# hdm0922/PathTracerDemo

Hardware: AMD Instinct MI355X
Metric: Msamples/sec at 1920x1080, 1 spp ReSTIR DI; per-pixel L2 vs WebGPU ref (higher is better)
Workload: dtype f32; 1 GPU; c3_interior_32 reuse 1920x1080, 1 spp/frame (configs[2]); frame=1920x1080, band_rows_per_gpu=1080, parallelism=row-bands x1

## Files before the change

### pathtracerdemo_amd/csrc/ptx_api.cpp

```cpp
#include <hip/hip_runtime.h>

#include <algorithm>
#include <cmath>
#include <cstdarg>
#include <cstdlib>
#include <cstdio>
#include <cstring>
#include <new>
#include <string>
#include <unordered_map>
#include <vector>

#include "ptx_internal.h"

namespace ptx {


[[maybe_unused]] static const char *const kShippedKnobs[] = {"COMM_TIMEOUT_S", "DEBUG_FILL", "HALO_PROXY_US"};
#if defined(PTX_WG_TIMES)
static const char *const kBuildKind = "wgt";
#elif defined(PTX_AB_BUILD)
static const char *const kBuildKind = "ab";
#else
static const char *const kBuildKind = "product";
// ... 758 lines not shown
                if (e != hipSuccess) break;
            }
            TimedLaunch *t = event_begin(h, PTX_STAT_WAVE_LOGIC, st);
            e = wave_gi_round(sc, w, gp, r, A, st);
            event_end(t, st);
        }
        return e;
    }
    if (pass == PTX_PASS_TEMPORAL || pass == PTX_PASS_SPATIAL || pass == kPassTemporalJobs ||
        pass == kPassTemporalCombine || is_motion_pass(pass)) {
        const bool temporal = pass != PTX_PASS_SPATIAL;
        ReuseArgs A = is_motion_pass(pass) ? motion_args(h)
                                           : reuse_args(h, temporal ? PTX_PASS_TEMPORAL : PTX_PASS_SPATIAL);
        WaveBufs wj = w;
        if (A.fold_last && wj.res[2]) wj.nres = 3;
        else A.fold_last = 0u;
        if (fused && pass == PTX_PASS_SPATIAL) {
            A.fuse_final = 1u;
            A.accum = (float4 *)h->d_accum.p;
            A.replay_cnt = (uint32_t *)h->d_replay.p;
            A.replay = A.replay_cnt + w.cnt_stride;
            A.replay_total = (unsigned long long *)h->d_counters.p + CNT_REPLAY;
        }
        const int nr = reuse_rounds(temporal, A);
        const int r_first = pass == kPassTemporalCombine ? nr + 1 : 0;
        const int r_last = pass == kPassTemporalJobs ? nr : nr + 1;
        for (int r = r_first; e == hipSuccess && r <= r_last; ++r) {
            if (r > 0 && r <= nr) {
                TimedLaunch *t = event_begin(h, PTX_STAT_WAVE_TRACE, st);
                e = wave_trace(sc, wj, r - 1, 1, h->stack_depth, st);
                event_end(t, st);
            }
            if (e != hipSuccess) break;
            if (r == nr && A.fold_last) continue;
            const bool combine = r == nr + 1 && pass == PTX_PASS_SPATIAL;
            if (combine && combine_after && (e = hipStreamWaitEvent(st, combine_after, 0)) != hipSuccess) break;
            TimedLaunch *t = event_begin(h, PTX_STAT_WAVE_LOGIC, st);
            e = wave_reuse_round(sc, wj, temporal, r, A, st);
            event_end(t, st);
            if (combine && combine_done && e == hipSuccess) e = hipEventRecord(combine_done, st);
        }
        return e;
    }
    const uint4 *fres = h->cfg.pipeline == PTX_PIPELINE_RESTIR_REUSE ? (const uint4 *)hist_band(h) : res;
    static const bool final_one = ab_knob("FINAL_ONE", 1) != 0;
    if (pass == PTX_PASS_FINAL && final_one && h->cfg.pipeline == PTX_PIPELINE_RESTIR_REUSE && tables_fit_lds(sc)) {
        TimedLaunch *t = event_begin(h, PTX_STAT_WAVE_LOGIC, st);
        if (fused)
            e = wave_final_replay(sc, w, gb, fres, acc, (const uint32_t *)h->d_replay.p + w.cnt_stride,
                                  (uint32_t *)h->d_replay.p, h->stack_depth, st);
        else
            e = wave_final_one(sc, w, gb, fres, acc, h->stack_depth, st);
        event_end(t, st);
        h->launches[PTX_STAT_FINAL_FUSED] += 1;
        h->cur().init_state_valid = false;
        return e;
    }
    h->cur().init_state_valid = pass == PTX_PASS_INIT && h->cfg.pipeline == PTX_PIPELINE_RESTIR_REUSE;
    const int rounds = pass == PTX_PASS_INIT ? kWaveRoundsInit : pass == PTX_PASS_FINAL ? kWaveRoundsFinal
                                                                                        : kWaveRoundsMcpt;
    for (int r = 0; e == hipSuccess && r <= rounds; ++r) {
        if (r > 0) {
            TimedLaunch *t = event_begin(h, PTX_STAT_WAVE_TRACE, st);
            e = wave_trace(sc, w, r - 1, 1, h->stack_depth, st);
            event_end(t, st);
        }
        if (e != hipSuccess) break;
// ... 59 lines not shown
    static const int env_bk = ab_knob("PIPE_BACK_STREAMS", 2);
    int k = env_bk > 0 && frames_in_flight(h) ? env_bk : 1;
    if (h->cfg.flags & PTX_FLAG_SINGLE_STREAM) k = 1;
    k = std::max(1, std::min<int>({k, ptx_handle::kMaxSplit, (int)interior.nseg, (int)edge.nseg}));
    ReuseArgs A = reuse_args(h, PTX_PASS_SPATIAL);
    const bool fold = A.fold_last && interior.res[2];
    if (!fold) A.fold_last = 0u;
    const int nr = reuse_rounds(0, A);
    if ((e = fork_sequences(h, k)) != hipSuccess) return e;
    const bool surf_stale = interior.surf && !h->cur().surf_valid;
    uint32_t E = 0u;
    for (int q = 0; q < k && e == hipSuccess; ++q) {
        hipStream_t st = q ? h->cur().sub[q] : h->cur().stream;
        WaveBufs wi = interior, we = edge;
        seg_share(wi, interior.nseg, q, k);
        seg_share(we, edge.nseg, q, k);
        wi.seg_phys = interior.seg_phys + E;
        we.seg_phys = interior.seg_phys + E + wi.seg_base + wi.seg_count - we.seg_base;
        E += we.seg_count;
        if (fold) wi.nres = we.nres = 3;
        WaveBufs wt = wi;
        wt.seg_count = wi.seg_count + we.seg_count;
        if (surf_stale) {
            if ((e = wave_surface(sc, wi, gbuf_band(h), st)) != hipSuccess) return e;
            if ((e = wave_surface(sc, we, gbuf_band(h), st)) != hipSuccess) return e;
        }
        for (int r = 0; e == hipSuccess && r <= nr + 1; ++r) {
            if (r > 0 && r <= nr) {
                TimedLaunch *t = event_begin(h, PTX_STAT_WAVE_TRACE, st);
                e = wave_trace(sc, wt, r - 1, 1, h->stack_depth, st);
                event_end(t, st);
                if (e != hipSuccess) break;
            }
            if (r == nr && A.fold_last) continue;
            TimedLaunch *t = event_begin(h, PTX_STAT_WAVE_LOGIC, st);
            e = wave_reuse_round(sc, wi, 0, r, A, st);
            if (e == hipSuccess && r == 0 && halo) e = hipStreamWaitEvent(st, halo, 0);
            if (e == hipSuccess) e = wave_reuse_round(sc, we, 0, r, A, st);
            event_end(t, st);
        }
        for (const WaveBufs *ws : {&wi, &we})
            if (e == hipSuccess) e = launch_wave_seq(h, sc, *ws, PTX_PASS_FINAL, st);
    }
    if (surf_stale && e == hipSuccess) h->cur().surf_valid = true;
    return e == hipSuccess ? join_sequences(h, k) : e;
}

hipError_t launch_wave_parts(ptx_handle *h, const Scene &sc, const WaveBufs &w, const int *passes, int npasses,
                             bool summaries, const WaveBufs *then, hipEvent_t then_wait, bool keep_gbuf) {
    h->hand_n = 0;
    static const bool overlap_start = ab_knob("OVERLAP_START", 1) != 0;
    if (then && overlap_start && npasses == 2 && passes[0] == PTX_PASS_SPATIAL && passes[1] == PTX_PASS_FINAL &&
        h->cfg.pipeline == PTX_PIPELINE_RESTIR_REUSE && !summaries)
        return spatial_overlap_seq(h, sc, w, *then, then_wait);
    static const int env_k = ab_knob("WAVE_STREAMS", 0);
    static const int env_pk = ab_knob("PIPE_STREAMS", 0);
    const bool band_h = h->comm || h->halo_top || h->halo_bot || (h->cfg.flags & PTX_FLAG_HALO_SKIP);
    const int pipe_k = env_pk > 0 ? env_pk : band_h || h->cfg.pipeline == PTX_PIPELINE_RESTIR_GI ? 1 : 2;
    int k = frames_in_flight(h) ? pipe_k : env_k > 0 ? env_k : 3;
    static const int env_bk = ab_knob("PIPE_BACK_STREAMS", 2);
    if (env_bk > 0 && frames_in_flight(h))
        for (int i = 0; i < npasses; ++i)
            if (passes[i] == PTX_PASS_SPATIAL) k = env_bk;
    if (h->cfg.flags & PTX_FLAG_SINGLE_STREAM) k = 1;
    k = std::max(1, std::min<int>(k, ptx_handle::kMaxSplit));
    if ((uint32_t)k > std::max(w.nseg, then ? then->nseg : 0u)) k = (int)std::max(w.nseg, then ? then->nseg : 0u);
    hipError_t e = hipSuccess;
// ... 2187 lines not shown
```

### pathtracerdemo_amd/csrc/ptx_reuse.hip

```cpp
#include "ptx_wave_common.h"

namespace ptx {

constexpr uint32_t SALT_TEMPORAL = 0x54454D50u, SALT_SPATIAL = 0x53504154u;

enum : uint32_t { JS_HDR, JS_F, JS_CUR, JS_NRM, JS_PREV, JS_RRF, JS_COUNT };
constexpr uint32_t kJobFresh = 1u << 24;
constexpr uint32_t kResReuseLayout = 0x100u;
#ifndef PTX_JOB_FRESH
#define PTX_JOB_FRESH 1
#endif

struct Job {
    uint32_t i, length, phase, seed1, idx, matref;
    uint32_t k, lab;
    bool shift, rok;
    int32_t ref;
    int32_t dom;
    f3 f;
    float prod;
    Surface cur;
    f3 prev;
    float beta, rr_p;
    f3 rr_f;
// ... 321 lines not shown
}
__device__ __forceinline__ float4 job_at(const ReuseArgs &A, const WaveBufs &w, uint32_t pix, uint32_t slot) {
    const uint32_t jid = job_id(A, pix, slot);
    return job_result(A, w, A.jres[jid], jid);
}
__device__ __forceinline__ SelF stored_f(const uint4 *r) {
    const uint4 r6 = r[6], r7 = r[7];
    return SelF{r7.w == 1u, mk(asf(r6.z), asf(r6.w), asf(r7.z))};
}
__device__ __forceinline__ uint32_t write_reused(uint4 *out, const uint4 *src, float p_sel, float q_sel, SelF fs,
                                                 float w_sum, uint32_t C) {
    uint4 a0 = src[0], a5 = src[5];
    const uint4 a1 = src[1], a2 = src[2], a3 = src[3], a4 = src[4];
    if (fs.known && !(a5.x & kResReuseLayout)) {
        const uint32_t k = a5.x & 0xffu;
        if (k >= 2u && k + 1u < a5.w) a0 = src[6];
        a5.x |= kResReuseLayout;
    }
    out[0] = a0; out[1] = a1; out[2] = a2; out[3] = a3; out[4] = a4; out[5] = a5;
    out[6] = make_uint4(asu(p_sel), asu(q_sel), fs.known ? asu(fs.f.x) : 0u, fs.known ? asu(fs.f.y) : 0u);
    out[7] = make_uint4(asu(p_sel > 0.0f ? w_sum / p_sel : 0.0f), C, fs.known ? asu(fs.f.z) : 0u, fs.known ? 1u : 0u);
    return a5.w;
}

constexpr uint32_t kNbrEscape = 0xFFFFFFFFu;
__device__ __forceinline__ uint4 nbr_pack(bool valid, uint4 r5, uint4 r6, uint4 r7) {
    uint32_t w = 0u;
    const uint32_t k = r5.x & 0xffu;
    if (valid)
        w = (r5.w > 0xfu || k > 0xfu || r7.y > 0x7ffffeu) ? kNbrEscape : (1u << 31) | (r5.w << 27) | (k << 23) | r7.y;
    return make_uint4(r6.x, r6.y, r7.x, w);
}

__device__ __forceinline__ bool temporal_from_init(const Scene &sc, const WaveBufs &w, const ReuseArgs &A, Job &s,
                                                   uint32_t pix, uint32_t jid) {
    const uint4 *rv = res_at(A.cur, s.ref);
    const bool hyb = job_hyb(s);
    while (s.i + 1u < s.length) {
        f3 V = normalize(s.prev - s.cur.pos);
        uint32_t seed = s.i == 1u ? rv[0].x : s.seed1, lobe;
        const f3 dir = sample_bsdf(seed, s.cur, V, lobe);
        float pdf;
        const f3 fv = bsdf_pdf(s.cur, V, dir, pdf);
        if (!hyb || s.i + 2u <= s.k) s.prod *= pdf;
        if (!rr_step(s, s.cur, dir, fv, pdf)) {
            A.jres[jid] = make_float4(0.0f, 0.0f, 0.0f, 0.0f);
            return false;
        }
        const float4 c = w.state[(s.i == 1u ? kStateCs2 : kStateCs3) * w.npix + pix];
        const Surface next = get_surface(sc, gdecode(make_uint4(asu(c.x), asu(c.y), asu(c.z), asu(c.w))));
        V = normalize(s.prev - s.cur.pos);
        const f3 L = normalize(next.pos - s.cur.pos);
        s.f = s.f * (bsdf(s.cur, L, V) * fabsf(dot(s.cur.nrm, L)));
        if (hyb && s.i + 1u == s.k) s.prod = s.prod * rc_geo(s.cur.pos, next);
        s.prev = s.cur.pos;
        s.cur = next;
        s.i += 1u;
    }
    const float T = w.state[kStateTsel * w.npix + pix].x;
    if (T < 0.0f) return true;
    const LightSample XL = load_xl(rv);
    const f3 V = normalize(s.prev - s.cur.pos);
    const f3 L = direction_to_light(s.cur, XL);
    s.f = s.f * (bsdf(s.cur, L, V) * fabsf(dot(s.cur.nrm, L)));
    float gl = 1.0f;
    if (XL.type == LIGHT_RECT) {
        const f3 r = XL.pos - s.cur.pos;
        const f3 Ld = normalize(r);
        gl = fabsf(dot(get_light(sc, (uint32_t)XL.id).dir, Ld)) / dot(r, r);
    }
    s.prod = hyb ? s.prod / s.beta : s.prod / (gl * s.beta);
    const f3 Le = l_emit<true>(XL, s.cur);
    s.f = s.f * (Le * T);
    const float qv = s.prod;
    const bool valid = qv > 0.0f && qv <= 3.402823466e38f;
    A.jres[jid] = valid ? make_float4(s.f.x, s.f.y, s.f.z, qv) : make_float4(0.0f, 0.0f, 0.0f, 0.0f);
    return false;
}

template <bool LDS_SHADE>
__global__ __launch_bounds__(WB) __attribute__((amdgpu_waves_per_eu(2, 8)))
void wtemporal_start(Scene gsc, WaveBufs w, ReuseArgs A) {
    PTX_WAVE_TIMER(gsc, KID_TEMP_START | (w.seg_base ? 0x80u : 0u));
    __shared__ uint32_t lds[3];
    extern __shared__ __attribute__((aligned(16))) uint32_t shade_lds[];
    const JobLists JL = job_lists(w, lds);
    const Scene sc = shading_scene<LDS_SHADE>(gsc, shade_lds, true);
    const Seg g = seg_begin(w, 0u, lds);
    const uint32_t np = padded_pixels(sc);
    for (uint32_t k = 0; k < w.seg_px; k += WB) {
        const uint32_t q = seg_pixel(w, g.j, k);
        uint32_t x, y, pix = 0u;
        bool active = false;
        Job s;
        if (q < np && tile_xy(sc, q, x, y)) {
            pix = (y - sc.row_begin) * sc.width + x;
            active = job_begin(sc, A, s, x, y, (int32_t)pix, (int32_t)pix);
            if (active && A.use_init) active = temporal_from_init(sc, w, A, s, pix, pix);
        }
        const bool live = job_emit(sc, g, A, active, s, pix, active ? A.cur[8u * (size_t)pix].x : 0u);
        job_finish(g, JL, A, live, s, pix);
    }
    job_seg_end(w, g, JL);
}

__global__ __launch_bounds__(WB) void wtemporal_combine(Scene sc, WaveBufs w, ReuseArgs A) {
    PTX_WAVE_TIMER(sc, KID_TEMP_COMBINE | (w.seg_base ? 0x80u : 0u));
    const uint32_t j = w.seg_base + blockIdx.x, np = padded_pixels(sc);
    for (uint32_t k = 0; k < w.seg_px; k += WB) {
        const uint32_t q = seg_pixel(w, j, k);
        uint32_t x, y;
        if (q >= np || !tile_xy(sc, q, x, y)) continue;
        const uint32_t pix = (y - sc.row_begin) * sc.width + x;
        if (!gdecode(A.gbuf[pix]).valid) {
            A.nbr_out[pix] = make_uint4(0u, 0u, 0u, 0u);
            continue;
        }
        uint4 *rv = A.cur + 8u * (size_t)pix;
        const uint4 *hv = A.hist + 8u * (size_t)pix;
        uint32_t seed = reuse_seed(sc, x, y, SALT_TEMPORAL);
        const uint4 r5 = rv[5], r7 = rv[7];
        const float4 er = (r7.y != 0u && r5.w >= 2u) ? job_result(A, w, A.jres[pix], pix) : make_float4(0.0f, 0.0f, 0.0f, 0.0f);
        const float2 ec = make_float2(er.w > 0.0f ? luminance(mk(er.x, er.y, er.z)) : 0.0f, er.w);
        const bool canon_ok = ec.y > 0.0f && ec.x > 0.0f;
        const uint4 h5 = hv[5], h6 = hv[6], h7 = hv[7];
        const uint32_t Cp = A.hist_valid ? min(h7.y, A.cap) : 0u;
        const float cp = (float)Cp, tot = 1.0f + cp;
        const float pp = asf(h6.x), qp = asf(h6.y);
        const bool hist_ok = Cp != 0u && h5.w >= 2u && pp > 0.0f;
        const float wc = canon_ok ? (1.0f / tot) * ec.x * asf(r7.x) : 0.0f;
        const float wp = hist_ok ? (cp / tot) * pp * asf(h7.x) : 0.0f;
        float w_sum = 0.0f, p_sel = ec.x, q_sel = ec.y;
        bool from_hist = false;
        if (wrs_update(w_sum, wc, seed)) { from_hist = false; p_sel = ec.x; q_sel = ec.y; }
        if (wrs_update(w_sum, wp, seed)) { from_hist = true; p_sel = pp; q_sel = qp; }
        write_reused(rv, from_hist ? hv : rv, p_sel, q_sel, from_hist ? stored_f(hv) : job_f(er), w_sum, 1u + Cp);
// ... 49 lines not shown
template <bool LDS_SHADE>
__global__ __launch_bounds__(WB) __attribute__((amdgpu_waves_per_eu(MOTION_START_WAVES, 8)))
void wtmotion_start(Scene gsc, WaveBufs w, ReuseArgs A) {
    PTX_WAVE_TIMER(gsc, KID_TEMP_START | (w.seg_base ? 0x80u : 0u));
    __shared__ uint32_t lds[3];
    extern __shared__ __attribute__((aligned(16))) uint32_t shade_lds[];
    const JobLists JL = job_lists(w, lds);
    const Scene sc = shading_scene<LDS_SHADE>(gsc, shade_lds, true);
    const Seg g = seg_begin(w, 0u, lds);
    const uint32_t np = padded_pixels(sc);
    for (uint32_t k = 0; k < w.seg_px; k += WB) {
        const uint32_t q = seg_pixel(w, g.j, k);
        uint32_t x = 0u, y = 0u, pix = 0u;
        bool valid = false;
        Surface X1{};
        uint32_t mref = 0u;
        if (q < np && tile_xy(sc, q, x, y)) {
            pix = (y - sc.row_begin) * sc.width + x;
            valid = surf_load(sc, A.surf, pix, X1, mref);
        }
        const uint4 *rv = A.cur + 8u * (size_t)pix;
        const uint4 r5c = valid ? rv[5] : make_uint4(0u, 0u, 0u, 0u);
        const uint32_t cC = valid ? rv[7].y : 0u, clen = r5c.w, ck = r5c.x & 0xffu;
        const bool canon = valid && cC != 0u && clen >= 2u;
        const MotionHist mh = valid ? motion_hist(sc, A, X1, y, true) : MotionHist{false, 0, 0u, 0u, 0u};
#pragma unroll 1
        for (uint32_t slot = 0; slot < kMotionJobs; ++slot) {
            const uint32_t jid = job_id(A, pix, slot);
            Job s;
            bool act = false;
            uint32_t s0 = 0u;
            if (slot == 0u) {
                act = canon && job_begin(sc, A, s, x, y, (int32_t)pix, (int32_t)pix);
                if (act && A.use_init) act = temporal_from_init(sc, w, A, s, pix, jid);
                if (act) s0 = rv[0].x;
            } else if (slot == 1u) {
                if (mh.ok) {
                    const uint4 *hv = A.hist + 8 * (ptrdiff_t)mh.pp;
                    const uint4 h0 = hv[0], h5 = hv[5], h6 = hv[6];
                    act = h5.w >= 2u && asf(h6.x) > 0.0f;
                    if (act) {
                        job_init(s, x0_of(sc, x, y), X1, mref, kHistRef + mh.pp, h5.w, h0.y, (int32_t)pix, h5.x & 0xffu,
                                 true);
                        s0 = h0.x;
                    }
                }
            } else if (mh.ok && canon) {
                Surface Xp;
                uint32_t pref;
                act = surf_load(sc, A.psurf, mh.pp, Xp, pref);
                if (act) {
                    job_init(s, x0_prev(A, sc, mh.px, mh.py), Xp, pref, (int32_t)pix, clen, rv[0].y, kDomPrev, ck, true);
                    s0 = rv[0].x;
                }
            }
            const bool live = job_emit(sc, g, A, act, s, jid, s0);
            job_finish(g, JL, A, live, s, jid);
        }
    }
    job_seg_end(w, g, JL);
}

__global__ __launch_bounds__(WB) void wtmotion_combine(Scene sc, WaveBufs w, ReuseArgs A) {
    PTX_WAVE_TIMER(sc, KID_TEMP_COMBINE | (w.seg_base ? 0x80u : 0u));
    const uint32_t j = w.seg_base + blockIdx.x, np = padded_pixels(sc);
    for (uint32_t k = 0; k < w.seg_px; k += WB) {
        const uint32_t q = seg_pixel(w, j, k);
// ... 502 lines not shown
                if (A.fuse_final) replay = shade_reused(sc, A, t, acc, pix, hit, hit ? Csum : 0u, length, fs, ucw);
            }
        }
        if (A.fuse_final) replay_append(A, w, w.seg_phys + j, replay, pix);
    }
}

__global__ __launch_bounds__(WB) void wspatial_combine(Scene sc, WaveBufs w, ReuseArgs A) {
    PTX_WAVE_TIMER(sc, KID_SPAT_COMBINE | (w.seg_base ? 0x80u : 0u));
    const uint32_t j = w.seg_base + blockIdx.x, np = padded_pixels(sc);
    for (uint32_t k = 0; k < w.seg_px; k += WB) {
        const uint32_t q = seg_pixel(w, j, k);
        uint32_t x, y, pix = 0u;
        bool replay = false;
        if (q < np && tile_xy(sc, q, x, y)) {
            pix = (y - sc.row_begin) * sc.width + x;
            if (!gdecode(A.gbuf[pix]).valid) {
                uint4 *out = A.hist + 8u * (size_t)pix;
                for (int t = 0; t < 8; ++t) out[t] = make_uint4(0u, 0u, 0u, 0u);
                if (A.fuse_final)
                    (void)shade_reused(sc, A, mix_weight(sc), A.accum[pix], pix, false, 0u, 0u,
                                       SelF{false, mk(0.0f, 0.0f, 0.0f)}, 0.0f);
            } else if (A.neighbors == 3u) {
                replay = combine_pixel<3>(sc, A, w, x, y, pix);
            } else {
                replay = combine_pixel<0>(sc, A, w, x, y, pix);
            }
        }
        if (A.fuse_final) replay_append(A, w, w.seg_phys + j, replay, pix);
    }
}

int reuse_rounds(int pass_temporal, const ReuseArgs &A) {
    return pass_temporal && A.use_init && !A.motion ? 1 : kWaveRoundsReuse;
}

hipError_t wave_reuse_round(const Scene &sc, const WaveBufs &w, int pass_temporal, int round, const ReuseArgs &A,
                            hipStream_t s) {
    const dim3 grid(w.seg_count), blk(WB);
    if (round == 0) {
        if (pass_temporal) {
            const bool staged = shade_from_lds(sc, SL_TEMPORAL_START);
            auto k = A.motion ? (staged ? wtmotion_start<true> : wtmotion_start<false>)
                              : (staged ? wtemporal_start<true> : wtemporal_start<false>);
            hipLaunchKernelGGL(k, grid, blk, shade_lds_bytes(staged, sc), s, sc, w, A);
        } else {
            hipLaunchKernelGGL(wspatial_start, grid, blk, 0, s, sc, w, A);
        }
    } else if (round <= reuse_rounds(pass_temporal, A)) {
        const bool staged = shade_from_lds(sc, SL_JOB_STEP);
        auto k = staged ? wjob_step<true> : wjob_step<false>;
        hipLaunchKernelGGL(k, grid, blk, shade_lds_bytes(staged, sc), s, sc, w, (uint32_t)round, A);
    } else {
        if (pass_temporal && A.motion) hipLaunchKernelGGL(wtmotion_combine, grid, blk, 0, s, sc, w, A);
        else if (pass_temporal) hipLaunchKernelGGL(wtemporal_combine, grid, blk, 0, s, sc, w, A);
        else if (A.neighbors == 3u && !ab_knob("COMBINE_SCALAR", 0))
            hipLaunchKernelGGL(wspatial_combine_shfl, dim3(w.seg_count), blk, 0, s, sc, w, A);
        else hipLaunchKernelGGL(wspatial_combine, grid, blk, 0, s, sc, w, A);
    }
    return hipGetLastError();
}

}
```

### pathtracerdemo_amd/csrc/ptx_wave.hip

```cpp
#include "ptx_stream.h"

#include <algorithm>
#include <cstdlib>

namespace ptx {

#ifndef TRACE_OCC_WAVES
#define TRACE_OCC_WAVES 5
#endif
template <bool COUNT, bool PROF, bool OCC, bool LDS_TABLES>
__device__ __forceinline__ void trace_lanes(const Scene &sc, const SubRoot *subs, const Inst *insts, PassEps eps,
                                            uint32_t *stack, CoopLds coop, Ray r, uint32_t kind, float T, float remain,
                                            uint32_t seg, bool active, float4 *res, uint32_t gi) {
    for (;;) {
        const float t_max = !active ? __builtin_nanf("") : kind != Q_CLOSEST ? vis_bound(remain) : 1e10f;
        const Hit h = (LDS_TABLES && !COUNT)
                          ? trace_core_flat<PROF, OCC>(sc, subs, insts, r, eps, stack, WB, t_max, coop, remain)
                          : trace_core_tab<COUNT, PROF, true, OCC, true>(sc, subs, insts, r, eps, stack, WB, t_max, coop,
                                                                         false, remain);
        if (active && end_query(sc, subs, insts, eps, h, r, kind, T, remain, seg, res, gi)) active = false;
        if (wballot(active) == 0ull) break;
    }
}
template <bool COUNT, bool PROF, bool OCC, bool LDS_TABLES>
// ... 165 lines not shown
                sp += 1;
            }
        }
    }
}

template <bool ROOTQ>
__global__ __launch_bounds__(WB) void wgbuffer(Scene sc, WaveBufs w, uint4 *gbuf) {
    PTX_WAVE_TIMER(sc, KID_GBUF);
    extern __shared__ __attribute__((aligned(16))) uint32_t wstack[];
    uint32_t *stack = wstack + tables_lds_bytes(sc) / 4u + threadIdx.x;
    const LdsTables T = stage_tables(sc, wstack);
    const uint32_t L = blockIdx.x * 4u + threadIdx.x / 64u, run = w.cluster * w.seg_count;
    const uint32_t t = set_tile(w, (L / run) * w.cluster * w.nseg + w.cluster * w.seg_base + L % run);
    const uint32_t q = t * 64u + (threadIdx.x & 63u);
    uint32_t x, y;
    if (q >= padded_pixels(sc) || !tile_xy(sc, q, x, y)) return;
    const float *vpinv = reinterpret_cast<const float *>(sc.U + U_VPINV);
    const float u = ((float)x + 0.5f) / (float)sc.U[U_W];
    const float v = ((float)y + 0.5f) / (float)sc.U[U_H];
    const f3 st = xform_point(vpinv, mk(2.0f * u - 1.0f, 2.0f * v - 1.0f, 0.0f));
    const f3 en = xform_point(vpinv, mk(2.0f * u - 1.0f, 2.0f * v - 1.0f, 0.0f + 1.0f));
    const Hit h = trace_core_tab<false, false, ROOTQ>(sc, T.subs, T.insts, Ray{st, normalize(en - st)},
                                                      PassEps{1e-8f, 1e-6f}, stack, WB);
    Compact c = h.s;
    c.valid = h.valid ? 1u : 0u;
    gbuf[(y - sc.row_begin) * sc.width + x] = gencode(c);
}

enum : uint32_t { IS_HDR, IS_FP, IS_RES, IS_X, IS_XL, IS_L, IS_BSEED, IS_CS2, IS_CS3, IS_TSEL, IS_COUNT };
static_assert(IS_CS2 == kStateCs2 && IS_CS3 == kStateCs3 && IS_TSEL == kStateTsel && IS_COUNT <= kWaveStateSlots,
              "PT_1 state slots read by the temporal pass (ptx_reuse.hip)");
enum : uint32_t { F_SEL = 1u, F_BSDF = 2u, F_FAR12 = 4u, F_FAR23 = 8u, F_R1 = 16u, F_R2 = 32u };

struct WInit {
    uint32_t seed, i, flags, C, vis_idx, bsdf_idx;
    f3 f; float p;
    float w_sum, p_hat_sel, pdf_env;
    f3 xpos; float xrough;
    f3 xlpos; uint32_t nee_seed;
    f3 L;
    uint32_t bseed1, bseed2;
};
__device__ __forceinline__ uint32_t lobe_of(uint32_t flags, uint32_t k) { return (flags >> (8u + 2u * (k - 1u))) & 3u; }

__device__ __forceinline__ void wcompress(const Scene &sc, const WInit &s, const float4 *state, uint32_t npix,
                                          uint32_t pix, bool is_env, const LightSample &XL, uint4 *out,
                                          bool rcnext) {
    const uint32_t i = s.i, length = i + 1u;
    const uint32_t L1 = (i > 1u || is_env) ? lobe_of(s.flags, 1u) : 0u;
    const uint32_t L2 = (i > 2u || (is_env && i == 2u)) ? lobe_of(s.flags, 2u) : 0u;
    const uint32_t s2 = (i >= 2u || is_env) ? s.bseed1 : s.nee_seed;
    const uint32_t s3 = (i >= 3u || (i == 2u && is_env)) ? s.bseed2 : (i == 2u ? s.nee_seed : 0u);
    const uint32_t s4 = (i == 3u) ? s.nee_seed : 0u;
    uint32_t k = 0u;
    if (length > 2u) {
        bool ok = (L1 == LOBE_LAMBERT || (s.flags & F_R1)) && (L2 == LOBE_LAMBERT || (s.flags & F_R2));
        if ((s.flags & F_FAR12) && ok) k = 2u;
    }
    if (k == 0u && length > 3u) {
        bool ok = (L2 == LOBE_LAMBERT || (s.flags & F_R2));
        if ((s.flags & F_FAR23) && ok) k = 3u;
    }
    if (k == 0u) {
        bool rough = s.xrough >= RECONNECTION_ROUGHNESS;
        bool dirl = XL.type == LIGHT_DIRECTION || XL.type == LIGHT_ENV;
        if ((dirl || length3(s.xpos - XL.pos) >= RECONNECTION_DISTANCE) && rough) k = length;
    }
    uint4 rc = make_uint4(0u, 0u, 0u, 0u);
    uint32_t lk = 0u, lk1 = 0u;
    if (k == length) {
        lk = LOBE_LIGHT;
        lk1 = (k == 2u) ? L1 : (k == 3u) ? L2 : 0u;
    } else if (k == 2u) {
        lk = L2; lk1 = L1;
        const float4 c = state[IS_CS2 * npix + pix];
        rc = make_uint4(asu(c.x), asu(c.y), asu(c.z), asu(c.w));
    } else if (k == 3u) {
        lk1 = L2;
        const float4 c = state[IS_CS3 * npix + pix];
        rc = make_uint4(asu(c.x), asu(c.y), asu(c.z), asu(c.w));
    }
    out[0] = make_uint4(s2, s3, s4, 0u);
    out[1] = make_uint4(asu(XL.dir.x), asu(XL.dir.y), asu(XL.dir.z), XL.type);
    out[2] = make_uint4(asu(XL.pos.x), asu(XL.pos.y), asu(XL.pos.z), (uint32_t)XL.id);
    out[3] = make_uint4(asu(XL.Le.x), asu(XL.Le.y), asu(XL.Le.z), asu(XL.pdf));
    out[4] = rc;
    out[5] = make_uint4(k, lk1, lk, length);
    uint4 nx = make_uint4(0u, 0u, 0u, 0u);
    if (rcnext && k == 2u && length == 4u) {
        const float4 c = state[IS_CS3 * npix + pix];
        nx = make_uint4(asu(c.x), asu(c.y), asu(c.z), asu(c.w));
    }
    out[6] = nx;
}

__device__ __forceinline__ void winit_vertex(const Scene &sc, const Seg &g, bool emit, WInit &s, const Surface &X,
                                             f3 prev) {
    float4 *rays = g.rays, *res = g.res_out;
    const uint32_t vbase = g.rbase + wave_alloc(g.l_ray, emit ? 1u : 0u);
    bool bsdf_ray = false;
    if (emit) {
        const f3 V = normalize(prev - X.pos);
        s.nee_seed = s.seed;
        const LightSample XL = sample_nee(sc, s.seed, X, V);
        const f3 Ln = direction_to_light(X, XL);
        f3 contrib = s.f * l_emit<false>(XL, X);
        contrib = contrib * bsdf(X, V, Ln);
        contrib = contrib * fabsf(dot(X.nrm, Ln));
        const float denom = s.p * XL.pdf;
        const float u_update = rnd(s.seed);
        s.xlpos = XL.pos;
        s.xpos = X.pos;
        s.xrough = X.mat.rough;
        s.vis_idx = vbase;
        const float dist = length(XL.pos - X.pos);
        put_ray(rays, vbase, X.pos, (XL.pos - X.pos) / dist, dist, Q_VIS);
        res[2u * vbase] = make_float4(0.0f, contrib.x, contrib.y, contrib.z);
        res[2u * vbase + 1u] = make_float4(denom, u_update, XL.pdf, asf((uint32_t)XL.id));
        if (s.i < 3u) {
            if (s.i == 1u) s.bseed1 = s.seed;
            else s.bseed2 = s.seed;
            uint32_t lobe;
            const f3 Lb = sample_bsdf(s.seed, X, V, lobe);
            s.flags |= lobe << (8u + 2u * (s.i - 1u));
            float pdfv;
            const f3 bv = bsdf_pdf(X, V, Lb, pdfv);
            s.f = s.f * (bv * fabsf(dot(X.nrm, Lb)));
            s.p *= pdfv;
            const float ps = luminance(s.f) / s.p;
            if (rnd(s.seed) < ps) {
                s.p *= ps;
                s.pdf_env = pdfv;
                s.L = Lb;
                bsdf_ray = true;
            }
        }
        s.flags = bsdf_ray ? (s.flags | F_BSDF) : (s.flags & ~F_BSDF);
    }
    const uint32_t bbase = g.rbase + wave_alloc(g.l_ray, bsdf_ray ? 1u : 0u);
    if (bsdf_ray) {
        s.bsdf_idx = bbase;
        put_ray(rays, bbase, s.xpos, s.L, -1.0f, Q_CLOSEST);
    }
}

__device__ __forceinline__ void winit_store(float4 *state, uint32_t npix, uint32_t pix, const WInit &s) {
    state[IS_HDR * npix + pix] = make_float4(asf(s.seed), asf(s.i | (s.flags << 8)), asf(s.C), asf(s.vis_idx));
    state[IS_FP * npix + pix] = make_float4(s.f.x, s.f.y, s.f.z, s.p);
    state[IS_RES * npix + pix] = make_float4(s.w_sum, s.p_hat_sel, s.pdf_env, asf(s.bsdf_idx));
    state[IS_X * npix + pix] = make_float4(s.xpos.x, s.xpos.y, s.xpos.z, s.xrough);
    state[IS_XL * npix + pix] = make_float4(s.xlpos.x, s.xlpos.y, s.xlpos.z, asf(s.nee_seed));
    state[IS_L * npix + pix] = make_float4(s.L.x, s.L.y, s.L.z, 0.0f);
    state[IS_BSEED * npix + pix] = make_float4(asf(s.bseed1), asf(s.bseed2), 0.0f, 0.0f);
}
__device__ __forceinline__ void winit_load(const float4 *state, uint32_t npix, uint32_t pix, WInit &s) {
    const float4 h = state[IS_HDR * npix + pix], fp = state[IS_FP * npix + pix], r = state[IS_RES * npix + pix];
    const float4 x = state[IS_X * npix + pix], xl = state[IS_XL * npix + pix], l = state[IS_L * npix + pix];
    const float4 b = state[IS_BSEED * npix + pix];
    s.seed = asu(h.x); s.i = asu(h.y) & 0xffu; s.flags = asu(h.y) >> 8; s.C = asu(h.z); s.vis_idx = asu(h.w);
    s.f = mk(fp.x, fp.y, fp.z); s.p = fp.w;
    s.w_sum = r.x; s.p_hat_sel = r.y; s.pdf_env = r.z; s.bsdf_idx = asu(r.w);
    s.xpos = mk(x.x, x.y, x.z); s.xrough = x.w;
    s.xlpos = mk(xl.x, xl.y, xl.z); s.nee_seed = asu(xl.w);
    s.L = mk(l.x, l.y, l.z);
    s.bseed1 = asu(b.x); s.bseed2 = asu(b.y);
}
__device__ __forceinline__ void winit_finish(const WInit &s, uint4 *reservoir, uint32_t pix) {
    uint4 *out = reservoir + 8u * (size_t)pix;
    if (!(s.flags & F_SEL))
        for (int q = 0; q < 7; ++q) out[q] = make_uint4(0u, 0u, 0u, 0u);
    out[7] = make_uint4(asu(s.w_sum / s.p_hat_sel), s.C, 0u, 0u);
}

template <bool LDS_SHADE>
__global__ __launch_bounds__(WB) __attribute__((amdgpu_waves_per_eu(LOGIC_WAVES, 8))) void winit_start(Scene gsc, WaveBufs w, const uint4 *gbuf, uint4 *reservoir) {
    PTX_WAVE_TIMER(gsc, KID_INIT_START | (w.seg_base ? 0x80u : 0u));
// ... 1 lines not shown
    extern __shared__ __attribute__((aligned(16))) uint32_t shade_lds[];
    const JobLists JL = job_lists(w, lds);
    const Scene sc = shading_scene<LDS_SHADE>(gsc, shade_lds, true);
    const Seg g = seg_begin(w, 0u, lds);
    float4 *state = w.state;
    const uint32_t npix = w.npix, np = padded_pixels(sc);
    for (uint32_t k = 0; k < w.seg_px; k += WB) {
        const uint32_t q = seg_pixel(w, g.j, k);
        uint32_t x, y, pix = 0u;
        bool active = false;
        WInit s;
        Surface X;
        f3 prev;
        if (q < np && tile_xy(sc, q, x, y)) {
            pix = (y - sc.row_begin) * sc.width + x;
            const Compact x1 = gdecode(gbuf[pix]);
            if (!x1.valid) {
                uint4 *out = reservoir + 8u * (size_t)pix;
                for (int q8 = 0; q8 < 8; ++q8) out[q8] = make_uint4(0u, 0u, 0u, 0u);
                if (w.surf) surf_store_none(w.surf, pix);
            } else {
                active = true;
                s.seed = pcg(x * 1973u + y * 9277u + sc.U[U_FRAME] * 26699u);
                s.i = 1u; s.flags = 0u; s.C = 0u;
                s.f = mk(1.0f, 1.0f, 1.0f); s.p = 1.0f;
                s.w_sum = 0.0f; s.p_hat_sel = 0.0f; s.pdf_env = 0.0f;
                s.L = mk(0.0f, 0.0f, 0.0f); s.bseed1 = 0u; s.bseed2 = 0u; s.bsdf_idx = 0u;
                prev = x0_of(sc, x, y);
                X = get_surface(sc, x1);
                if (w.surf) surf_store(w.surf, pix, X, mat_index(sc, x1.inst, x1.mat));
                if (X.mat.rough >= RECONNECTION_ROUGHNESS) s.flags |= F_R1;
            }
        }
        winit_vertex(sc, g, active, s, X, prev);
        if (active) winit_store(state, npix, pix, s);
        job_keep(g, JL, active, active && !(s.flags & F_BSDF), pix);
    }
    job_seg_end(w, g, JL);
}

template <bool LDS_SHADE>
__global__ __launch_bounds__(WB) __attribute__((amdgpu_waves_per_eu(LOGIC_WAVES, 8))) void winit_step(Scene gsc, WaveBufs w, uint32_t round, uint4 *reservoir) {
    PTX_WAVE_TIMER(gsc, KID_INIT_STEP | (w.seg_base ? 0x80u : 0u));
    __shared__ uint32_t lds[3];
    extern __shared__ __attribute__((aligned(16))) uint32_t shade_lds[];
    const JobLists JL = job_lists(w, lds);
    const Scene sc = shading_scene<LDS_SHADE>(gsc, shade_lds, seg_n_in(w, round) != 0u);
    const Seg g = seg_begin(w, round, lds);
    float4 *state = w.state;
    const float4 *res_in = g.res_in;
    const uint32_t npix = w.npix;
    uint32_t nh;
    const uint32_t n = split_count(g, nh);
    for (uint32_t base = 0; base < n; base += WB) {
        const uint32_t q = base + threadIdx.x;
        bool emit = false;
        uint32_t pix = 0u;
        WInit s;
        Surface X;
        f3 prev;
        if (q < n) {
            pix = split_at(g, JL, q, nh);
            winit_load(state, npix, pix, s);
            const float4 a = res_in[2u * s.vis_idx], b = res_in[2u * s.vis_idx + 1u];
            const f3 contrib = mk(a.y, a.z, a.w) * a.x;
            const float p_hat = luminance(contrib);
            const float ris = p_hat / b.x;
            s.C += 1u;
            s.w_sum += ris;
            if (b.y < ris / s.w_sum) {
                s.flags |= F_SEL;
                s.p_hat_sel = p_hat;
                state[IS_TSEL * npix + pix] = make_float4(a.x, 0.0f, 0.0f, 0.0f);
                LightSample XL;
                const Light ls = get_light(sc, asu(b.w));
                XL.id = (int32_t)asu(b.w);
                XL.type = ls.type;
                XL.Le = ls.color * ls.intensity;
                XL.pos = s.xlpos;
                XL.pdf = b.z;
                XL.dir = ls.type == LIGHT_DIRECTION ? ls.dir
                         : ls.type == LIGHT_POINT  ? normalize(s.xpos - ls.pos)
                         : ls.type == LIGHT_RECT   ? normalize(s.xpos - s.xlpos)
                                                   : mk(0.0f, 0.0f, 0.0f);
                wcompress(sc, s, state, npix, pix, false, XL, reservoir + 8u * (size_t)pix, w.surf != nullptr);
            }
            if (!(s.flags & F_BSDF)) {
                winit_finish(s, reservoir, pix);
            } else {
                const Hit h = get_hit(res_in, s.bsdf_idx);
                if (!h.valid) {
                    const float u = rnd(s.seed);
                    const float ph = luminance(s.f * ENV_C);
                    const float ris_e = ph / s.p;
                    s.C += 1u;
                    s.w_sum += ris_e;
                    if (u < ris_e / s.w_sum) {
                        s.flags |= F_SEL;
                        s.p_hat_sel = ph;
                        state[IS_TSEL * npix + pix] = make_float4(-1.0f, 0.0f, 0.0f, 0.0f);
                        LightSample env;
                        env.pos = s.xpos + s.L * INF_F;
                        env.type = LIGHT_ENV;
                        env.dir = -s.L;
                        env.id = -1;
                        env.Le = mk(ENV_C, ENV_C, ENV_C);
                        env.pdf = s.pdf_env;
                        wcompress(sc, s, state, npix, pix, true, env, reservoir + 8u * (size_t)pix, w.surf != nullptr);
                    }
                    winit_finish(s, reservoir, pix);
                } else {
                    X = surface_at(sc, h.s, h.pos);
                    prev = s.xpos;
                    s.i += 1u;
                    if (s.i == 2u) {
                        if (length3(prev - X.pos) >= RECONNECTION_DISTANCE) s.flags |= F_FAR12;
                        if (X.mat.rough >= RECONNECTION_ROUGHNESS) s.flags |= F_R2;
                        const uint4 e = gencode(h.s);
                        state[IS_CS2 * npix + pix] = make_float4(asf(e.x), asf(e.y), asf(e.z), asf(e.w));
                    } else {
                        if (length3(prev - X.pos) >= RECONNECTION_DISTANCE) s.flags |= F_FAR23;
                        const uint4 e = gencode(h.s);
                        state[IS_CS3 * npix + pix] = make_float4(asf(e.x), asf(e.y), asf(e.z), asf(e.w));
                    }
                    emit = true;
                }
            }
        }
        winit_vertex(sc, g, emit, s, X, prev);
        if (emit) winit_store(state, npix, pix, s);
        job_keep(g, JL, emit, emit && !(s.flags & F_BSDF), pix);
    }
    job_seg_end(w, g, JL);
}

enum : uint32_t { FS_HDR, FS_F, FS_CUR, FS_NRM, FS_PREV, FS_COUNT };

struct WFinal {
    uint32_t i, length, phase, seed1, idx;
    f3 f; float ucw;
    Surface cur;
    f3 prev;
};
__device__ __forceinline__ void wfinal_emit(const Scene &sc, const Seg &g, bool emit, WFinal &s, const uint4 *resv) {
    float4 *rays = g.rays, *res = g.res_out;
    const uint32_t idx = g.rbase + wave_alloc(g.l_ray, emit ? 1u : 0u);
    if (!emit) return;
    const f3 V = normalize(s.prev - s.cur.pos);
    s.idx = idx;
    if (s.i + 1u < s.length) {
        uint32_t seed = s.i == 1u ? resv[0].x : s.seed1;
        uint32_t lobe;
        const f3 dir = sample_bsdf(seed, s.cur, V, lobe);
        s.phase = 0u;
        put_ray(rays, idx, s.cur.pos, dir, -1.0f, Q_CLOSEST);
    } else {
        const LightSample XL = load_xl(resv);
        const f3 L = direction_to_light(s.cur, XL);
        s.f = s.f * (bsdf(s.cur, L, V) * fabsf(dot(s.cur.nrm, L)));
        const f3 Le = l_emit<true>(XL, s.cur);
        s.phase = 1u;
        const float dist = length(XL.pos - s.cur.pos);
        put_ray(rays, idx, s.cur.pos, (XL.pos - s.cur.pos) / dist, dist, Q_VIS);
        res[2u * idx] = make_float4(0.0f, Le.x, Le.y, Le.z);
// ... 542 lines not shown
```

Before: 575.8 Msamples/s.

## Book env-escape visibility during init and drop temporal reuse trace round

When an init path escapes to the environment, the init pass now emits a visibility ray for the env sample and stores its result in the selected-light slot on a later step, so the temporal shift no longer has to trace. The temporal-from-init path therefore runs zero trace rounds. A dedicated non-compacting kernel variant with a higher waves-per-EU hint evaluates the shift directly per pixel. This removes one trace launch and the job-list compaction machinery, at the cost of extra rays in the init pass and a new packed-flag encoding in the job lists.

```diff
diff --git a/pathtracerdemo_amd/csrc/ptx_api.cpp b/pathtracerdemo_amd/csrc/ptx_api.cpp
--- a/pathtracerdemo_amd/csrc/ptx_api.cpp
+++ b/pathtracerdemo_amd/csrc/ptx_api.cpp
@@ -814,7 +814,7 @@
                 event_end(t, st);
             }
             if (e != hipSuccess) break;
-            if (r == nr && A.fold_last) continue;
+            if (r > 0 && r == nr && A.fold_last) continue;
             const bool combine = r == nr + 1 && pass == PTX_PASS_SPATIAL;
             if (combine && combine_after && (e = hipStreamWaitEvent(st, combine_after, 0)) != hipSuccess) break;
             TimedLaunch *t = event_begin(h, PTX_STAT_WAVE_LOGIC, st);
@@ -940,7 +940,7 @@
                 event_end(t, st);
                 if (e != hipSuccess) break;
             }
-            if (r == nr && A.fold_last) continue;
+            if (r > 0 && r == nr && A.fold_last) continue;
             TimedLaunch *t = event_begin(h, PTX_STAT_WAVE_LOGIC, st);
             e = wave_reuse_round(sc, wi, 0, r, A, st);
             if (e == hipSuccess && r == 0 && halo) e = hipStreamWaitEvent(st, halo, 0);
diff --git a/pathtracerdemo_amd/csrc/ptx_reuse.hip b/pathtracerdemo_amd/csrc/ptx_reuse.hip
--- a/pathtracerdemo_amd/csrc/ptx_reuse.hip
+++ b/pathtracerdemo_amd/csrc/ptx_reuse.hip
@@ -377,7 +377,7 @@
     return make_uint4(r6.x, r6.y, r7.x, w);
 }
 
-__device__ __forceinline__ bool temporal_from_init(const Scene &sc, const WaveBufs &w, const ReuseArgs &A, Job &s,
+__device__ __forceinline__ void temporal_from_init(const Scene &sc, const WaveBufs &w, const ReuseArgs &A, Job &s,
                                                    uint32_t pix, uint32_t jid) {
     const uint4 *rv = res_at(A.cur, s.ref);
     const bool hyb = job_hyb(s);
@@ -390,7 +390,7 @@
         if (!hyb || s.i + 2u <= s.k) s.prod *= pdf;
         if (!rr_step(s, s.cur, dir, fv, pdf)) {
             A.jres[jid] = make_float4(0.0f, 0.0f, 0.0f, 0.0f);
-            return false;
+            return;
         }
         const float4 c = w.state[(s.i == 1u ? kStateCs2 : kStateCs3) * w.npix + pix];
         const Surface next = get_surface(sc, gdecode(make_uint4(asu(c.x), asu(c.y), asu(c.z), asu(c.w))));
@@ -403,10 +403,15 @@
         s.i += 1u;
     }
     const float T = w.state[kStateTsel * w.npix + pix].x;
-    if (T < 0.0f) return true;
     const LightSample XL = load_xl(rv);
     const f3 V = normalize(s.prev - s.cur.pos);
     const f3 L = direction_to_light(s.cur, XL);
+    bool ok = true;
+    if (XL.type == LIGHT_ENV) {
+        float pdf;
+        const f3 fv = bsdf_pdf(s.cur, V, L, pdf);
+        ok = rr_step(s, s.cur, L, fv, pdf);
+    }
     s.f = s.f * (bsdf(s.cur, L, V) * fabsf(dot(s.cur.nrm, L)));
     float gl = 1.0f;
     if (XL.type == LIGHT_RECT) {
@@ -418,35 +423,50 @@
     const f3 Le = l_emit<true>(XL, s.cur);
     s.f = s.f * (Le * T);
     const float qv = s.prod;
-    const bool valid = qv > 0.0f && qv <= 3.402823466e38f;
+    const bool valid = ok && qv > 0.0f && qv <= 3.402823466e38f;
     A.jres[jid] = valid ? make_float4(s.f.x, s.f.y, s.f.z, qv) : make_float4(0.0f, 0.0f, 0.0f, 0.0f);
-    return false;
-}
-
-template <bool LDS_SHADE>
-__global__ __launch_bounds__(WB) __attribute__((amdgpu_waves_per_eu(2, 8)))
+}
+
+#ifndef TEMPORAL_INIT_WAVES
+#define TEMPORAL_INIT_WAVES 4
+#endif
+template <bool LDS_SHADE, bool FROM_INIT>
+__global__ __launch_bounds__(WB) __attribute__((amdgpu_waves_per_eu(FROM_INIT ? TEMPORAL_INIT_WAVES : 2, 8)))
 void wtemporal_start(Scene gsc, WaveBufs w, ReuseArgs A) {
     PTX_WAVE_TIMER(gsc, KID_TEMP_START | (w.seg_base ? 0x80u : 0u));
-    __shared__ uint32_t lds[3];
     extern __shared__ __attribute__((aligned(16))) uint32_t shade_lds[];
-    const JobLists JL = job_lists(w, lds);
-    const Scene sc = shading_scene<LDS_SHADE>(gsc, shade_lds, true);
-    const Seg g = seg_begin(w, 0u, lds);
-    const uint32_t np = padded_pixels(sc);
-    for (uint32_t k = 0; k < w.seg_px; k += WB) {
-        const uint32_t q = seg_pixel(w, g.j, k);
-        uint32_t x, y, pix = 0u;
-        bool active = false;
-        Job s;
-        if (q < np && tile_xy(sc, q, x, y)) {
-            pix = (y - sc.row_begin) * sc.width + x;
-            active = job_begin(sc, A, s, x, y, (int32_t)pix, (int32_t)pix);
-            if (active && A.use_init) active = temporal_from_init(sc, w, A, s, pix, pix);
-        }
-        const bool live = job_emit(sc, g, A, active, s, pix, active ? A.cur[8u * (size_t)pix].x : 0u);
-        job_finish(g, JL, A, live, s, pix);
-    }
-    job_seg_end(w, g, JL);
+    if constexpr (FROM_INIT) {
+        const Scene sc = shading_scene<LDS_SHADE>(gsc, shade_lds, true);
+        if constexpr (LDS_SHADE) __syncthreads();
+        const uint32_t j = w.seg_base + blockIdx.x, np = padded_pixels(sc);
+        for (uint32_t k = 0; k < w.seg_px; k += WB) {
+            const uint32_t q = seg_pixel(w, j, k);
+            uint32_t x, y;
+            if (q >= np || !tile_xy(sc, q, x, y)) continue;
+            const uint32_t pix = (y - sc.row_begin) * sc.width + x;
+            Job s;
+            if (job_begin(sc, A, s, x, y, (int32_t)pix, (int32_t)pix)) temporal_from_init(sc, w, A, s, pix, pix);
+        }
+    } else {
+        __shared__ uint32_t lds[3];
+        const JobLists JL = job_lists(w, lds);
+        const Scene sc = shading_scene<LDS_SHADE>(gsc, shade_lds, true);
+        const Seg g = seg_begin(w, 0u, lds);
+        const uint32_t np = padded_pixels(sc);
+        for (uint32_t k = 0; k < w.seg_px; k += WB) {
+            const uint32_t q = seg_pixel(w, g.j, k);
+            uint32_t x, y, pix = 0u;
+            bool active = false;
+            Job s;
+            if (q < np && tile_xy(sc, q, x, y)) {
+                pix = (y - sc.row_begin) * sc.width + x;
+                active = job_begin(sc, A, s, x, y, (int32_t)pix, (int32_t)pix);
+            }
+            const bool live = job_emit(sc, g, A, active, s, pix, active ? A.cur[8u * (size_t)pix].x : 0u);
+            job_finish(g, JL, A, live, s, pix);
+        }
+        job_seg_end(w, g, JL);
+    }
 }
 
 __global__ __launch_bounds__(WB) void wtemporal_combine(Scene sc, WaveBufs w, ReuseArgs A) {
@@ -562,7 +582,10 @@
             uint32_t s0 = 0u;
             if (slot == 0u) {
                 act = canon && job_begin(sc, A, s, x, y, (int32_t)pix, (int32_t)pix);
-                if (act && A.use_init) act = temporal_from_init(sc, w, A, s, pix, jid);
+                if (act && A.use_init) {
+                    temporal_from_init(sc, w, A, s, pix, jid);
+                    act = false;
+                }
                 if (act) s0 = rv[0].x;
             } else if (slot == 1u) {
                 if (mh.ok) {
@@ -1131,7 +1154,7 @@
 }
 
 int reuse_rounds(int pass_temporal, const ReuseArgs &A) {
-    return pass_temporal && A.use_init && !A.motion ? 1 : kWaveRoundsReuse;
+    return pass_temporal && A.use_init && !A.motion ? 0 : kWaveRoundsReuse;
 }
 
 hipError_t wave_reuse_round(const Scene &sc, const WaveBufs &w, int pass_temporal, int round, const ReuseArgs &A,
@@ -1140,8 +1163,9 @@
     if (round == 0) {
         if (pass_temporal) {
             const bool staged = shade_from_lds(sc, SL_TEMPORAL_START);
-            auto k = A.motion ? (staged ? wtmotion_start<true> : wtmotion_start<false>)
-                              : (staged ? wtemporal_start<true> : wtemporal_start<false>);
+            auto k = A.motion    ? (staged ? wtmotion_start<true> : wtmotion_start<false>)
+                     : A.use_init ? (staged ? wtemporal_start<true, true> : wtemporal_start<false, true>)
+                                  : (staged ? wtemporal_start<true, false> : wtemporal_start<false, false>);
             hipLaunchKernelGGL(k, grid, blk, shade_lds_bytes(staged, sc), s, sc, w, A);
         } else {
             hipLaunchKernelGGL(wspatial_start, grid, blk, 0, s, sc, w, A);
diff --git a/pathtracerdemo_amd/csrc/ptx_wave.hip b/pathtracerdemo_amd/csrc/ptx_wave.hip
--- a/pathtracerdemo_amd/csrc/ptx_wave.hip
+++ b/pathtracerdemo_amd/csrc/ptx_wave.hip
@@ -221,6 +221,8 @@
 static_assert(IS_CS2 == kStateCs2 && IS_CS3 == kStateCs3 && IS_TSEL == kStateTsel && IS_COUNT <= kWaveStateSlots,
               "PT_1 state slots read by the temporal pass (ptx_reuse.hip)");
 enum : uint32_t { F_SEL = 1u, F_BSDF = 2u, F_FAR12 = 4u, F_FAR23 = 8u, F_R1 = 16u, F_R2 = 32u };
+constexpr uint32_t kEnvWait = 0x80000000u;
+static_assert(kWaveRoundsInit == 3, "an env escape (steps 1, 2) is followed by a step that books its Visibility");
 
 struct WInit {
     uint32_t seed, i, flags, C, vis_idx, bsdf_idx;
@@ -284,10 +286,10 @@
     out[6] = nx;
 }
 
-__device__ __forceinline__ void winit_vertex(const Scene &sc, const Seg &g, bool emit, WInit &s, const Surface &X,
-                                             f3 prev) {
+__device__ __forceinline__ uint32_t winit_vertex(const Scene &sc, const Seg &g, bool emit, WInit &s, const Surface &X,
+                                                 f3 prev, bool spare = false) {
     float4 *rays = g.rays, *res = g.res_out;
-    const uint32_t vbase = g.rbase + wave_alloc(g.l_ray, emit ? 1u : 0u);
+    const uint32_t vbase = g.rbase + wave_alloc(g.l_ray, emit || spare ? 1u : 0u);
     bool bsdf_ray = false;
     if (emit) {
         const f3 V = normalize(prev - X.pos);
@@ -332,6 +334,7 @@
         s.bsdf_idx = bbase;
         put_ray(rays, bbase, s.xpos, s.L, -1.0f, Q_CLOSEST);
     }
+    return vbase;
 }
 
 __device__ __forceinline__ void winit_store(float4 *state, uint32_t npix, uint32_t pix, const WInit &s) {
@@ -399,7 +402,7 @@
                 if (X.mat.rough >= RECONNECTION_ROUGHNESS) s.flags |= F_R1;
             }
         }
-        winit_vertex(sc, g, active, s, X, prev);
+        (void)winit_vertex(sc, g, active, s, X, prev);
         if (active) winit_store(state, npix, pix, s);
         job_keep(g, JL, active, active && !(s.flags & F_BSDF), pix);
     }
@@ -419,15 +422,21 @@
     const uint32_t npix = w.npix;
     uint32_t nh;
     const uint32_t n = split_count(g, nh);
+    const bool reuse = w.surf != nullptr;
     for (uint32_t base = 0; base < n; base += WB) {
         const uint32_t q = base + threadIdx.x;
-        bool emit = false;
+        bool emit = false, env_vis = false;
         uint32_t pix = 0u;
         WInit s;
         Surface X;
         f3 prev;
-        if (q < n) {
-            pix = split_at(g, JL, q, nh);
+        const uint32_t ent = q < n ? split_at(g, JL, q, nh) : 0u;
+        if (q < n && (ent & kEnvWait)) {
+            pix = ent & ~kEnvWait;
+            const float4 t = state[IS_TSEL * npix + pix];
+            state[IS_TSEL * npix + pix] = make_float4(res_in[2u * asu(t.y)].x, 0.0f, 0.0f, 0.0f);
+        } else if (q < n) {
+            pix = ent;
             winit_load(state, npix, pix, s);
             const float4 a = res_in[2u * s.vis_idx], b = res_in[2u * s.vis_idx + 1u];
             const f3 contrib = mk(a.y, a.z, a.w) * a.x;
@@ -465,7 +474,8 @@
                     if (u < ris_e / s.w_sum) {
                         s.flags |= F_SEL;
                         s.p_hat_sel = ph;
-                        state[IS_TSEL * npix + pix] = make_float4(-1.0f, 0.0f, 0.0f, 0.0f);
+                        if (!reuse) state[IS_TSEL * npix + pix] = make_float4(-1.0f, 0.0f, 0.0f, 0.0f);
+                        env_vis = reuse;
                         LightSample env;
                         env.pos = s.xpos + s.L * INF_F;
                         env.type = LIGHT_ENV;
@@ -494,9 +504,15 @@
                 }
             }
         }
-        winit_vertex(sc, g, emit, s, X, prev);
+        const uint32_t eidx = winit_vertex(sc, g, emit, s, X, prev, env_vis);
         if (emit) winit_store(state, npix, pix, s);
-        job_keep(g, JL, emit, emit && !(s.flags & F_BSDF), pix);
+        if (env_vis) {
+            const f3 xl = s.xpos + s.L * INF_F;
+            const float dist = length(xl - s.xpos);
+            put_ray(g.rays, eidx, s.xpos, (xl - s.xpos) / dist, dist, Q_VIS);
+            state[IS_TSEL * npix + pix] = make_float4(-1.0f, asf(eidx), 0.0f, 0.0f);
+        }
+        job_keep(g, JL, emit || env_vis, env_vis || (emit && !(s.flags & F_BSDF)), env_vis ? pix | kEnvWait : pix);
     }
     job_seg_end(w, g, JL);
 }
```

Result: no change. 577.7 Msamples/s (median of 6 runs) (+0.3%).
